# codeslake/RefVSR

Hardware: AMD Instinct MI355X
Metric: 4x SR frames/sec (270p->1080p, RefVSR_small_L1) (higher is better)
Workload: dtype f16; 1 GPU; config_RefVSR_small_L1 4x SR, 270x480 -> 1080x1920, frame_num=5, steady-state sliding window, n=1 (BASELINE configs[1]); synthetic clip seed 0, seeded random weights 1234; frames_per_rank=20, parallelism=frame-shard x1 (reset-aligned, no collective), window_cache=True, frame_ids=True, pipelined_calls=True, frames_per_call=4, headline_mode=frame groups, pipe_layout=pfm, full=False

## Files before the change

### refvsr_amd/csrc/common.h

```cpp
#pragma once
#include <stdlib.h>
#include <hip/hip_runtime.h>
#include <hip/hip_fp16.h>
#include <stdint.h>
#include <stdio.h>
#include <string.h>
#include <type_traits>
#include <utility>

#include "../../include/refvsr_hip.h"

typedef _Float16 f16;
typedef f16 f16x2 __attribute__((ext_vector_type(2)));
typedef f16 f16x4 __attribute__((ext_vector_type(4)));
typedef f16 f16x8 __attribute__((ext_vector_type(8)));
typedef float f32x4 __attribute__((ext_vector_type(4)));
typedef float f32x16 __attribute__((ext_vector_type(16)));

void refvsr_set_error(const char* fmt, ...);

#define RV_CHECK(cond, ...)                        \
    do {                                           \
        if (!(cond)) {                             \
            refvsr_set_error(__VA_ARGS__);         \
            return 1;                              \
        }                                          \
    } while (0)

#define RV_HIP(call)                                                                  \
    do {                                                                              \
        hipError_t e_ = (call);                                                       \
        if (e_ != hipSuccess) {                                                       \
            refvsr_set_error("%s failed: %s (%s:%d)", #call, hipGetErrorString(e_), __FILE__, __LINE__); \
            return 2;                                                                 \
        }                                                                             \
    } while (0)

#define RV_LAUNCH_CHECK() RV_HIP(hipGetLastError())

static inline int rv_cdiv(int a, int b) { return (a + b - 1) / b; }

template <class F, int... I>
__device__ __forceinline__ void rv_static_for(F&& f, std::integer_sequence<int, I...>) { (f(std::integral_constant<int, I>{}), ...); }

#define RV_MAX_DEVICES 16
static inline int rv_device() {
    int d = 0;
    if (hipGetDevice(&d) != hipSuccess || d < 0 || d >= RV_MAX_DEVICES) d = 0;
    return d;
}
static inline int rv_num_cus() {
    static int n_cu[RV_MAX_DEVICES] = {};
    const int d = rv_device();
    if (n_cu[d] == 0) {
        hipDeviceProp_t prop;
        if (hipGetDeviceProperties(&prop, d) == hipSuccess) n_cu[d] = prop.multiProcessorCount;
        if (n_cu[d] <= 0) n_cu[d] = 256;
    }
    return n_cu[d];
}

int rv_stream_cus(hipStream_t st);

struct RvLaunchCap {
    bool attr_done[RV_MAX_DEVICES];
    int occ[RV_MAX_DEVICES];
    size_t occ_lds[RV_MAX_DEVICES];
};
template <typename Kernel>
static int rv_launch_cap(RvLaunchCap& c, Kernel kernel, int block, size_t attr_lds, size_t lds, hipStream_t st, int* cap) {
    const int dev = rv_device();
    if (!c.attr_done[dev]) {
        RV_HIP(hipFuncSetAttribute(reinterpret_cast<const void*>(kernel), hipFuncAttributeMaxDynamicSharedMemorySize, (int)attr_lds));
        c.attr_done[dev] = true;
    }
    if (block == 0) {
        c.occ[dev] = 1;
    } else if (c.occ[dev] == 0 || c.occ_lds[dev] != lds) {
        int occ = 0;
        RV_HIP(hipOccupancyMaxActiveBlocksPerMultiprocessor(&occ, kernel, block, lds));
        c.occ[dev] = occ < 1 ? 1 : occ;
        c.occ_lds[dev] = lds;
    }
    *cap = (rv_stream_cus(st) * c.occ[dev]) & ~7;
    if (*cap < 8) *cap = 8;
    return 0;
}

template <typename Args, typename Launch>
static int rv_resblock_chain(const char* name, int pxb, int min_blob, const void* const* src, int batch, int h, int w, int n,
                             const void* blobs, size_t blob_stride, float act_slope, void* scratch0, void* scratch1, void* const* out,
                             void* stream, Launch launch) {
    RV_CHECK(src && out && blobs && h > 0 && w > 0 && n >= 1 && batch >= 1 && batch <= REFVSR_MAX_MAPS, "%s: bad args", name);
    RV_CHECK(blob_stride >= (size_t)min_blob && blob_stride % 16 == 0 && ((uintptr_t)blobs & 15) == 0,
             "%s: blobs must be 16-byte aligned, stride >= %d", name, min_blob);
    RV_CHECK(act_slope >= 0.f && act_slope <= 1.f, "%s: activation slope must lie in [0, 1]", name);
    RV_CHECK(n == 1 || scratch0, "%s: n >= 2 needs scratch0", name);
    RV_CHECK(n <= 2 || scratch1, "%s: n >= 3 needs scratch1", name);
    const size_t mapb = (size_t)h * w * pxb;
    for (int b = 0; b < batch; ++b) {
        RV_CHECK(src[b] && out[b], "%s: null map pointer (map %d)", name, b);
        for (int c = 0; c < batch; ++c) {
            const unsigned char* s0 = scratch0 ? (const unsigned char*)scratch0 + c * mapb : nullptr;
            const unsigned char* s1 = scratch1 ? (const unsigned char*)scratch1 + c * mapb : nullptr;
            RV_CHECK(src[b] != out[c] && s0 != out[b] && s1 != out[b] && (n < 2 || s0 != src[b]) && (n < 3 || s1 != src[b]) &&
                     (c == b || out[b] != out[c]), "%s: buffers must be distinct", name);
        }
    }
    RV_CHECK(n < 3 || scratch0 != scratch1, "%s: buffers must be distinct", name);
    RV_CHECK((long long)h * w * pxb < (1ll << 31), "%s: map too large for 32-bit offsets", name);
    RV_CHECK(refvsr_init() == 0, "init failed");
    Args a;
    memset(&a, 0, sizeof(a));
    a.h = h; a.w = w; a.act_slope = act_slope; a.batch = batch;
    hipStream_t st = (hipStream_t)stream;
    const unsigned char* cur[REFVSR_MAX_MAPS];
    for (int b = 0; b < batch; ++b) cur[b] = (const unsigned char*)src[b];
    for (int i = 0; i < n; ++i) {
        unsigned char* sc = (unsigned char*)((i & 1) ? scratch1 : scratch0);
        for (int b = 0; b < batch; ++b) {
            a.bsrc[b] = cur[b];
            a.bout[b] = (i == n - 1) ? (unsigned char*)out[b] : sc + b * mapb;
        }
        a.src = a.bsrc[0]; a.out = a.bout[0]; a.blob = (const unsigned char*)blobs + (size_t)i * blob_stride;
        const int rc = launch(a, st);
        if (rc) return rc;
        for (int b = 0; b < batch; ++b) cur[b] = a.bout[b];
    }
    return 0;
}

__device__ __forceinline__ void rv_tile_range(const int n_tiles, const int g, int& t_begin, int& t_end) {
    const int b = (int)blockIdx.x;
    int rank = b;
    if (g >= 8) {
        const int xcd = b & 7;
        rank = b >> 3;
        for (int y = 0; y < xcd; ++y) rank += (g - y + 7) >> 3;
    }
    const unsigned un = (unsigned)n_tiles, ug = (unsigned)g;
    t_begin = (int)(((unsigned)rank * un) / ug);
    t_end = (int)(((unsigned)(rank + 1) * un) / ug);
}

__device__ __forceinline__ int rv_reflect(int i, int n) {
    i = i < 0 ? -i : i;
    return i >= n ? 2 * (n - 1) - i : i;
}

__device__ __forceinline__ float rv_lrelu(float v, float slope) { return v >= 0.f ? v : v * slope; }

__device__ __forceinline__ float rv_linspace_m1p1(int j, int n) {
    const float step = 2.0f / (float)(n - 1);
    return (j < n / 2) ? (-1.0f + step * (float)j) : (1.0f - step * (float)(n - 1 - j));
}

struct WarpCoord { int x0, y0; float w00, w01, w10, w11; bool v00, v01, v10, v11; };

__device__ __forceinline__ WarpCoord warp_coord_uv(const float u, const float v, int hf, int wf, int hin, int win, int y, int x);
__device__ __forceinline__ WarpCoord warp_coord(const float* flow, int hf, int wf, int hin, int win, int y, int x) {
    const size_t fp = (size_t)y * wf + x;
    return warp_coord_uv(flow[fp], flow[(size_t)hf * wf + fp], hf, wf, hin, win, y, x);
}
__device__ __forceinline__ WarpCoord warp_coord_uv(const float u, const float v, int hf, int wf, int hin, int win, int y, int x) {
    const float gx = rv_linspace_m1p1(x, wf) + u / (((float)win - 1.0f) / 2.0f);
    const float gy = rv_linspace_m1p1(y, hf) + v / (((float)hin - 1.0f) / 2.0f);
    const float xs = ((gx + 1.0f) * (float)win - 1.0f) / 2.0f;
    const float ys = ((gy + 1.0f) * (float)hin - 1.0f) / 2.0f;
    const float fx = floorf(xs), fy = floorf(ys);
    const float tx = xs - fx, ty = ys - fy;
    WarpCoord c;
    c.x0 = (int)fminf(fmaxf(fx, -2.0f), (float)win + 1.0f);
    c.y0 = (int)fminf(fmaxf(fy, -2.0f), (float)hin + 1.0f);
    const bool xin0 = c.x0 >= 0 && c.x0 < win, xin1 = c.x0 + 1 >= 0 && c.x0 + 1 < win;
    const bool yin0 = c.y0 >= 0 && c.y0 < hin, yin1 = c.y0 + 1 >= 0 && c.y0 + 1 < hin;
    c.v00 = xin0 && yin0; c.v01 = xin1 && yin0; c.v10 = xin0 && yin1; c.v11 = xin1 && yin1;
    c.w00 = (1.0f - ty) * (1.0f - tx); c.w01 = (1.0f - ty) * tx;
    c.w10 = ty * (1.0f - tx); c.w11 = ty * tx;
    return c;
}

__device__ __forceinline__ uint4 warp_group16(const unsigned char* x, int pixb, int hin, int win, const WarpCoord& c, int goff) {
    float acc[8] = {0, 0, 0, 0, 0, 0, 0, 0};
    auto tap = [&](bool valid, int yy, int xx, float wgt) {
        if (valid) {
            const f16x8 v = *reinterpret_cast<const f16x8*>(x + ((size_t)yy * win + xx) * pixb + goff);
#pragma unroll
            for (int k = 0; k < 8; ++k) acc[k] += wgt * (float)v[k];
        }
    };
    tap(c.v00, c.y0, c.x0, c.w00);
    tap(c.v01, c.y0, c.x0 + 1, c.w01);
    tap(c.v10, c.y0 + 1, c.x0, c.w10);
    tap(c.v11, c.y0 + 1, c.x0 + 1, c.w11);
    union { f16x8 h; uint4 u; } o;
#pragma unroll
    for (int k = 0; k < 8; ++k) o.h[k] = (f16)acc[k];
    return o.u;
}

__device__ __forceinline__ void rv_bilinear_ac_src(int o, int n_in, int n_out, int& i0, int& i1, float& l1) {
#pragma clang fp contract(off)
    const float sc = n_out > 1 ? (float)(n_in - 1) / (float)(n_out - 1) : 0.0f;
    const float x = (float)o * sc;
    i0 = min((int)x, n_in - 1);
    i1 = min(i0 + 1, n_in - 1);
    l1 = x - (float)i0;
}
__device__ __forceinline__ float rv_bilinear_ac2_at(const float* __restrict__ s, int h, int w, int oy, int ox) {
    int y0, y1, x0, x1;
    float ly, lx;
    rv_bilinear_ac_src(oy, h, 2 * h, y0, y1, ly);
    rv_bilinear_ac_src(ox, w, 2 * w, x0, x1, lx);
    const float wy0 = 1.0f - ly, wx0 = 1.0f - lx;
    const float r0 = fmaf(lx, s[(size_t)y0 * w + x1], fmaf(wx0, s[(size_t)y0 * w + x0], 0.0f));
    const float r1 = fmaf(lx, s[(size_t)y1 * w + x1], fmaf(wx0, s[(size_t)y1 * w + x0], 0.0f));
    return fmaf(ly, r1, fmaf(wy0, r0, 0.0f));
}

__device__ __forceinline__ void rv_cubic_taps(float t, float* wgt) {
    const float A = -0.75f;
    float x = t + 1.0f;
    wgt[0] = ((A * x - 5.0f * A) * x + 8.0f * A) * x - 4.0f * A;
    x = t;
    wgt[1] = ((A + 2.0f) * x - (A + 3.0f)) * x * x + 1.0f;
    x = 1.0f - t;
    wgt[2] = ((A + 2.0f) * x - (A + 3.0f)) * x * x + 1.0f;
    x = 2.0f - t;
    wgt[3] = ((A * x - 5.0f * A) * x + 8.0f * A) * x - 4.0f * A;
}
__device__ __forceinline__ void rv_cubic_src(int o, int n_in, float scale, int* idx, float* wgt) {
    const float x = ((float)o + 0.5f) * scale - 0.5f;
    const float fl = floorf(x);
    const int ix = (int)fl;
    rv_cubic_taps(x - fl, wgt);
#pragma unroll
    for (int k = 0; k < 4; ++k) idx[k] = min(max(ix - 1 + k, 0), n_in - 1);
}
__device__ __forceinline__ float rv_bicubic_at(const float* __restrict__ s, int h, int w, int oy, int ox, float sy, float sx) {
    int iy[4], ix[4];
    float wy[4], wx[4];
    rv_cubic_src(oy, h, sy, iy, wy);
    rv_cubic_src(ox, w, sx, ix, wx);
    float acc = 0.0f;
#pragma unroll
    for (int j = 0; j < 4; ++j) {
        float r = 0.0f;
        const float* row = s + (size_t)iy[j] * w;
#pragma unroll
        for (int i = 0; i < 4; ++i) r = fmaf(wx[i], row[ix[i]], r);
        acc = fmaf(wy[j], r, acc);
    }
    return acc;
}

__device__ __forceinline__ void rv_store_result(void* out, const size_t e, const float v, const int fmt) {
    const int f = fmt & REFVSR_RESULT_FMT_MASK;
    if (f == REFVSR_RESULT_F32) reinterpret_cast<float*>(out)[e] = v;
    else if (f == REFVSR_RESULT_F16) reinterpret_cast<f16*>(out)[e] = (f16)v;
    else reinterpret_cast<unsigned char*>(out)[e] = (unsigned char)__float2int_rn(v * 255.0f);
}
__host__ __device__ __forceinline__ size_t rv_result_index(const int fmt, const int c, const int y, const int x, const int h, const int w) {
    return (fmt & REFVSR_RESULT_HWC) ? ((size_t)y * w + x) * 3 + c : ((size_t)c * h + y) * w + x;
}
static inline bool rv_result_fmt_ok(const int fmt) {
    return fmt >= 0 && (fmt & ~(REFVSR_RESULT_FMT_MASK | REFVSR_RESULT_HWC)) == 0 && (fmt & REFVSR_RESULT_FMT_MASK) <= REFVSR_RESULT_U8;
}

__host__ __device__ inline int rv_keven(int ks, int ncg) {
    const int ce = (ncg + 1) >> 1, co = ncg >> 1;
    return ks * (((ks + 1) >> 1) * ce + (ks >> 1) * co);
}
__host__ __device__ inline int rv_ksteps(int ks, int ncg) { return (ks * ks * ncg + (rv_keven(ks, ncg) & 1) + 3) / 4; }
__host__ __device__ inline int rv_kslot(int ty, int tx, int cg, int ks, int ncg) {
    const int ce = (ncg + 1) >> 1, co = ncg >> 1;
    const int p = (tx + cg) & 1;
    const int c0 = p ? co : ce, c1 = p ? ce : co;
    const int row = ((ks + 1) >> 1) * c0 + (ks >> 1) * c1;
    const int rank = ty * row + ((tx + 1) >> 1) * c0 + (tx >> 1) * c1 + (cg >> 1);
    if (!p) return rank;
    const int E = rv_keven(ks, ncg);
    return E + (E & 1) + rank;
}
__host__ __device__ inline int rv_kpad_slot(int j, int ks, int ncg) {
    const int E = rv_keven(ks, ncg);
    return ((E & 1) && j == 0) ? E : ks * ks * ncg + j;
}
__device__ __forceinline__ int rv_pix16(int n) { return (n < 4 || n >= 12) ? ((n & 7) << 1) : (((n - 4) << 1) | 1); }
```

### refvsr_amd/csrc/conv24.hip

```cpp
#include "common.h"
#include "conv24_plan.h"
#include <stdlib.h>

struct C24Args {
    const unsigned char* src0; const unsigned char* src1; unsigned char* out;
    const unsigned char* blob; const unsigned char* mul; const unsigned char* res;
    int h, w, tiles_x, n_tiles, grid;
    float act_slope, post_slope;
    const float* conf_a; const float* conf_b;
    const float* cw0; const float* cb0;
    float* conf_max;
    int ch, cw;
    float slope0;
    const float* base_lr; int bh, bw; float base_step;
    int out_fmt;
    int batch, tpm;
    const unsigned char* bsrc0[REFVSR_MAX_MAPS]; const unsigned char* bsrc1[REFVSR_MAX_MAPS]; unsigned char* bout[REFVSR_MAX_MAPS];
    const unsigned char* bmul[REFVSR_MAX_MAPS]; const unsigned char* bres[REFVSR_MAX_MAPS];
    const float* bconf_a[REFVSR_MAX_MAPS]; const float* bconf_b[REFVSR_MAX_MAPS]; float* bconf_max[REFVSR_MAX_MAPS];
};

constexpr int c24_nf(int cout, int wf) { return wf ? (cout == 24 ? 2 : cout / 16) : cout == 24 ? 3 : cout == 3 ? 1 : cout / 8; }

__device__ __forceinline__ float c24_fold1(const float a) {
    const unsigned u = __float_as_uint(a);
    const auto pr = __builtin_amdgcn_permlane32_swap(u, u, false, false);
    const unsigned x0 = pr[0], x1 = pr[1];
    return __uint_as_float(x0) + __uint_as_float(x1);
}

template <int COUT, int NCG0, int NCG1, int NWV, int TH, int WPS, int SHUF = 0, int CONF = 0, int HALF = 0, int MM = 0, int WF = 0>
__global__ __launch_bounds__(NWV * 64) __attribute__((amdgpu_waves_per_eu(WPS, WPS))) void conv24_kernel(C24Args p) {
    static_assert(WF == 0 || COUT != 3, "output head: one fragment in either format");
    static_assert(HALF == 0 || (COUT == 24 && SHUF == 0 && CONF == 0), "channel-half variant: 24 computed channels per workgroup");
    static_assert(MM == 0 || (HALF == 0 && COUT != 3), "multi-map variant");
    static_assert(SHUF == 0 || (COUT == 48 && (SHUF == 24 || SHUF == 48) && NCG0 * 8 == SHUF && NCG1 == 0), "pixel-shuffle variant");
    static_assert(CONF == 0 || (NCG0 == 2 && NCG1 == 0 && SHUF == 0), "confidence variant: 16-channel single source");
    constexpr int NCG = NCG0 + NCG1, PS = NCG | 1, PXB = PS * 16, ROWB = C24_XW * PXB;
    constexpr int S = c24_steps(NCG), NPAT = c24_npat(NCG);
    constexpr int NF = c24_nf(COUT, WF);
    constexpr int NM = COUT == 24 ? 2 : COUT == 3 ? 1 : COUT / 16;
    constexpr int BIASB = COUT == 48 ? 256 : 128;
    constexpr int WB = S * NF * 1024, BIAS = WB, XT = WB + BIASB;
    constexpr int NT = NWV * 64, T = 2 * TH / NWV;
    constexpr int C24_TH = TH, C24_XH = TH + 2, C24_NPX = C24_XH * C24_XW;
    constexpr int NCH = C24_NPX * NCG, KCH = (NCH + NT - 1) / NT;
    constexpr int PIXB0 = NCG0 * 16, PIXB1 = NCG1 * 16;
    constexpr int OPX = HALF ? 96 : COUT * 2;
    static_assert((COUT == 3 || COUT == 24 || COUT == 32 || COUT == 48) && S > 0 && T >= 1 && T * NWV == 2 * TH, "unsupported shape");
    static_assert(COUT != 3 || (NCG1 == 0 && SHUF == 0 && CONF == 0), "output head: single source");
    extern __shared__ __attribute__((aligned(16))) unsigned char smem[];

    asm volatile("" :: "s"(p.src0), "s"(p.src1), "s"(p.out), "s"(p.blob), "s"(p.mul), "s"(p.res), "s"(p.h), "s"(p.w), "s"(p.tiles_x),
                 "s"(p.n_tiles), "s"(p.grid), "s"(p.act_slope), "s"(p.post_slope));
    const int tid = threadIdx.x;
    const int lane = tid & 63;
    const int wave = __builtin_amdgcn_readfirstlane(tid >> 6);

    {
        constexpr int NPC = WB / 1024;
        const unsigned char* g = p.blob + ((SHUF || HALF) ? (int)blockIdx.y * (WB + BIASB) : 0) + lane * 16;
#pragma unroll
        for (int j = 0; j < (NPC + NWV - 1) / NWV; ++j) {
            const int c = wave + j * NWV;
            if (c < NPC)
                __builtin_amdgcn_global_load_lds((const __attribute__((address_space(1))) void*)(g + c * 1024),
                                                 (__attribute__((address_space(3))) void*)(smem + c * 1024), 16, 0, 0);
        }
        if (wave == NPC % NWV && lane < BIASB / 16)
            __builtin_amdgcn_global_load_lds((const __attribute__((address_space(1))) void*)(g + NPC * 1024),
                                             (__attribute__((address_space(3))) void*)(smem + NPC * 1024), 16, 0, 0);
    }

    if constexpr (HALF != 0) {
        const int zoff = (int)blockIdx.y * 48;
        p.out += zoff;
        if (p.mul) p.mul += zoff;
        if (p.res) p.res += zoff;
    }
    const int rowp = p.w;
    unsigned xg[KCH], xl[KCH];
    unsigned xs1 = 0;
#pragma unroll
    for (int k = 0; k < KCH; ++k) {
        const int i = min(tid + k * NT, NCH - 1);
        const int px = i / NCG, cg = i - px * NCG;
        const int r = px / C24_XW, c = px - r * C24_XW;
        const bool s1 = cg >= NCG0;
        xg[k] = (unsigned)((r * rowp + c) * (s1 ? PIXB1 : PIXB0) + (s1 ? cg - NCG0 : cg) * 16);
        xl[k] = (unsigned)(XT + px * PXB + cg * 16);
        xs1 |= s1 ? (1u << k) : 0u;
    }
    uint4 xv[KCH];
    auto x_fetch = [&](const int tf) {
        int t = tf;
        const unsigned char* s0p = p.src0;
        const unsigned char* s1p = p.src1;
        if constexpr (MM != 0) {
            const int bm = (int)((unsigned)tf / (unsigned)p.tpm);
            t = tf - bm * p.tpm;
            s0p = p.bsrc0[bm];
            if constexpr (NCG1 != 0) s1p = p.bsrc1[bm];
        }
        const int tyi = t / p.tiles_x;
        const int ty0 = tyi * C24_TH, tx0 = (t - tyi * p.tiles_x) * C24_TW;
        const bool interior = ty0 >= 1 && ty0 + C24_TH + 1 <= p.h && tx0 >= 1 && tx0 + C24_TW + 1 <= p.w;
        const long long org = (long long)(ty0 - 1) * p.w + (tx0 - 1);
        const unsigned char* b0 = s0p + org * PIXB0;
        const unsigned char* b1 = NCG1 ? s1p + org * PIXB1 : b0;
        if (interior) {
#pragma unroll
            for (int k = 0; k < KCH; ++k)
                xv[k] = *reinterpret_cast<const uint4*>((NCG1 && ((xs1 >> k) & 1) ? b1 : b0) + xg[k]);
        } else {
            int tide = tid;
            asm volatile("" : "+v"(tide));
#pragma unroll
            for (int k = 0; k < KCH; ++k) {
                const int i = min(tide + k * NT, NCH - 1);
                const int px = i / NCG, cg = i - px * NCG;
                const int r = px / C24_XW, c = px - r * C24_XW;
                const int iy = ty0 - 1 + r, ix = tx0 - 1 + c;
                const bool ok = (unsigned)iy < (unsigned)p.h && (unsigned)ix < (unsigned)p.w;
                const bool s1 = cg >= NCG0;
                const unsigned pix = (unsigned)(min(max(iy, 0), p.h - 1) * p.w + min(max(ix, 0), p.w - 1));
                const unsigned char* g = s1 ? s1p + pix * PIXB1 + (cg - NCG0) * 16 : s0p + pix * PIXB0 + cg * 16;
                uint4 v = *reinterpret_cast<const uint4*>(g);
                const unsigned keep = ok ? 0xffffffffu : 0u;
                v.x &= keep; v.y &= keep; v.z &= keep; v.w &= keep;
                xv[k] = v;
            }
        }
    };
    auto x_park = [&]() {
#pragma unroll
        for (int k = 0; k < KCH; ++k)
            if (k * NT + NT <= NCH || tid + k * NT < NCH) *reinterpret_cast<uint4*>(smem + xl[k]) = xv[k];
    };
    constexpr int PTH = TH + 4, PTW = C24_XW + 2;
    constexpr int PT = XT + C24_NPX * PXB, CW0 = PT + 2 * PTH * PTW * 4, CB0 = CW0 + 18 * 16 * 4;
    if constexpr (CONF != 0) {
        float* wl0 = reinterpret_cast<float*>(smem + CW0);
        for (int i = tid; i < 18 * 16; i += NT) {
            const int co = i & 15, tap = i >> 4;
            wl0[i] = p.cw0[(co * 2 + tap / 9) * 9 + tap % 9];
        }
        if (tid < 16) reinterpret_cast<float*>(smem + CB0)[tid] = p.cb0[tid];
    }
    auto conf_stage = [&](const int tf) {
        int t = tf;
        const float* cap = p.conf_a;
        const float* cbp = p.conf_b;
        float* cmp_ = p.conf_max;
        if constexpr (MM != 0) {
            const int bm = (int)((unsigned)tf / (unsigned)p.tpm);
            t = tf - bm * p.tpm;
            cap = p.bconf_a[bm]; cbp = p.bconf_b[bm];
            if (p.conf_max) cmp_ = p.bconf_max[bm];
        }
        const int tyi = t / p.tiles_x;
        const int ty0 = tyi * C24_TH, tx0 = (t - tyi * p.tiles_x) * C24_TW;
        float* pt = reinterpret_cast<float*>(smem + PT);
        for (int i = tid; i < 2 * PTH * PTW; i += NT) {
            const int c = i / (PTH * PTW), rem = i - c * (PTH * PTW);
            const int r = rem / PTW, cc = rem - r * PTW;
            const int y = ty0 - 2 + r, x = tx0 - 2 + cc;
            float v = 0.0f;
            if ((unsigned)y < (unsigned)p.h && (unsigned)x < (unsigned)p.w) {
                const float* src = c ? cbp : cap;
                if constexpr (CONF == 1) v = src[(size_t)y * p.cw + x];
                else v = fminf(fmaxf(rv_bicubic_at(src, p.ch, p.cw, y, x, 0.5f, 0.5f), 0.0f), 1.0f);
            }
            pt[i] = v;
        }
        __syncthreads();
        const float* wl0 = reinterpret_cast<const float*>(smem + CW0);
        const float* bl0 = reinterpret_cast<const float*>(smem + CB0);
#pragma unroll
        for (int k = 0; k < KCH; ++k) {
            const int i = tid + k * NT;
            if (i < NCH) {
                const int px = i >> 1, cg = i & 1;
                const int r = px / C24_XW, c = px - r * C24_XW;
                const int iy = ty0 - 1 + r, ix = tx0 - 1 + c;
                uint4 v = make_uint4(0u, 0u, 0u, 0u);
                if ((unsigned)iy < (unsigned)p.h && (unsigned)ix < (unsigned)p.w) {
                    float acc[8] = {0.f, 0.f, 0.f, 0.f, 0.f, 0.f, 0.f, 0.f};
#pragma unroll
                    for (int ci = 0; ci < 2; ++ci)
#pragma unroll
                        for (int ky = 0; ky < 3; ++ky)
#pragma unroll
                            for (int kx = 0; kx < 3; ++kx) {
                                const float xv = pt[ci * (PTH * PTW) + (r + ky) * PTW + (c + kx)];
                                const f32x4 w0 = *reinterpret_cast<const f32x4*>(wl0 + (ci * 9 + ky * 3 + kx) * 16 + cg * 8);
                                const f32x4 w1 = *reinterpret_cast<const f32x4*>(wl0 + (ci * 9 + ky * 3 + kx) * 16 + cg * 8 + 4);
                                acc[0] = fmaf(xv, w0[0], acc[0]); acc[1] = fmaf(xv, w0[1], acc[1]);
                                acc[2] = fmaf(xv, w0[2], acc[2]); acc[3] = fmaf(xv, w0[3], acc[3]);
                                acc[4] = fmaf(xv, w1[0], acc[4]); acc[5] = fmaf(xv, w1[1], acc[5]);
                                acc[6] = fmaf(xv, w1[2], acc[6]); acc[7] = fmaf(xv, w1[3], acc[7]);
                            }
                    union { f16x8 h; uint4 u; } o;
#pragma unroll
                    for (int j = 0; j < 8; ++j) o.h[j] = (f16)rv_lrelu(acc[j] + bl0[cg * 8 + j], p.slope0);
                    v = o.u;
                }
                *reinterpret_cast<uint4*>(smem + XT + px * PXB + cg * 16) = v;
            }
        }
        if constexpr (CONF == 1) {
            if (p.conf_max) {
                for (int i = tid; i < C24_TH * C24_TW; i += NT) {
                    const int r = i / C24_TW, c = i - r * C24_TW;
                    const int y = ty0 + r, x = tx0 + c;
                    if (y < p.h && x < p.w)
                        cmp_[(size_t)y * p.w + x] = fmaxf(pt[(r + 2) * PTW + c + 2], pt[PTH * PTW + (r + 2) * PTW + c + 2]);
                }
            }
        }
    };
    int tl, k_hi;
    rv_tile_range(p.n_tiles, p.grid, tl, k_hi);
    if constexpr (CONF == 0) { if (tl < k_hi) x_fetch(tl); }
    __builtin_amdgcn_sched_barrier(0);

    const int q = lane >> 4;
    const int lp = rv_pix16(lane & 15);
    const int la = lane * 16;
    const int g0w = wave * T;
#define RW(t) ((g0w + (t)) >> 1)
#define CG(t) ((g0w + (t)) & 1)
    auto sel4 = [&](const int v0, const int v1, const int v2, const int v3) { return q == 0 ? v0 : q == 1 ? v1 : q == 2 ? v2 : v3; };
    int pb[T];
#pragma unroll
    for (int t = 0; t < T; ++t)
        pb[t] = XT + RW(t) * ROWB + (CG(t) * 16 + lp) * PXB +
                sel4(c24_off(NCG, 0, 0), c24_off(NCG, 0, 1), c24_off(NCG, 0, 2), c24_off(NCG, 0, 3)) - c24_off(NCG, 0, 0);
    int pd[NPAT];
#pragma unroll
    for (int pp = 0; pp < NPAT; ++pp) {
        const int s = c24_pat_step(NCG, pp);
        pd[pp] = (sel4(c24_off(NCG, s, 0), c24_off(NCG, s, 1), c24_off(NCG, s, 2), c24_off(NCG, s, 3)) - c24_off(NCG, s, 0)) -
                 (sel4(c24_off(NCG, 0, 0), c24_off(NCG, 0, 1), c24_off(NCG, 0, 2), c24_off(NCG, 0, 3)) - c24_off(NCG, 0, 0));
    }
    const int rowb_o = p.w * OPX;
    const unsigned oo = (unsigned)(lp * OPX + q * 8);

    if constexpr (CONF == 0) { if (tl < k_hi) x_park(); }
    __syncthreads();

    for (; tl < k_hi; ++tl) {
        const bool has_next = tl + 1 < k_hi;
        if constexpr (CONF != 0) {
            conf_stage(tl);
            __syncthreads();
        }
        int tm = tl;
        unsigned char* outp = p.out;
        const unsigned char* mulp = p.mul;
        const unsigned char* resp = p.res;
        if constexpr (MM != 0) {
            const int bm = (int)((unsigned)tl / (unsigned)p.tpm);
            tm = tl - bm * p.tpm;
            outp = p.bout[bm];
            if (p.mul) mulp = p.bmul[bm];
            if (p.res) resp = p.bres[bm];
        }
        const int tyi = tm / p.tiles_x;
        const int ty0 = tyi * C24_TH, tx0 = (tm - tyi * p.tiles_x) * C24_TW;
        const bool interior = ty0 >= 1 && ty0 + C24_TH + 1 <= p.h && tx0 >= 1 && tx0 + C24_TW + 1 <= p.w;
        const long long oorg = ((long long)ty0 * p.w + tx0) * OPX;
        f16x4 mv[NM][T], rv[NM][T];
        bool okt[T];
#pragma unroll
        for (int t = 0; t < T; ++t) {
            okt[t] = true;
            if (!interior) {
                int lpe = lp;
                asm volatile("" : "+v"(lpe));
                okt[t] = ty0 + RW(t) < p.h && tx0 + CG(t) * 16 + lpe < p.w;
            }
            const unsigned eo = (unsigned)(RW(t) * rowb_o) + oo + CG(t) * 16 * OPX;
#pragma unroll
            for (int m = 0; m < NM; ++m) {
                mv[m][t] = rv[m][t] = (f16x4){(f16)0.f, (f16)0.f, (f16)0.f, (f16)0.f};
                const bool lane_ok = okt[t] && (COUT != 24 || m == 0 || q < 2);
                if constexpr (COUT == 24) {
                    if (p.mul && lane_ok) mv[m][t] = *reinterpret_cast<const f16x4*>(mulp + oorg + eo + 32 * m);
                    if (p.res && lane_ok) rv[m][t] = *reinterpret_cast<const f16x4*>(resp + oorg + eo + 32 * m);
                }
                (void)lane_ok;
            }
        }
        if constexpr (CONF == 0) { if (has_next) x_fetch(tl + 1); }

        f32x4 acc[NM][T];
#pragma unroll
        for (int m = 0; m < NM; ++m) {
            const f32x4 bv = *reinterpret_cast<const f32x4*>(smem + BIAS + m * 64 + q * 16);
#pragma unroll
            for (int t = 0; t < T; ++t) acc[m][t] = bv;
        }
        {
            uint4 fa[2][NF], fb[2][T];
            auto load = [&](auto sc, uint4 (&af)[NF], uint4 (&bf)[T]) {
                constexpr int s = decltype(sc)::value;
                constexpr int pp = c24_pat(NCG, s);
                constexpr int imm = c24_off(NCG, s, 0);
#pragma unroll
                for (int f = 0; f < NF; ++f) af[f] = *reinterpret_cast<const uint4*>(smem + (s * NF + f) * 1024 + la);
#pragma unroll
                for (int t = 0; t < T; ++t) {
                    if constexpr (pp == 0) bf[t] = *reinterpret_cast<const uint4*>(smem + pb[t] + imm);
                    else bf[t] = *reinterpret_cast<const uint4*>(smem + pb[t] + pd[pp] + imm);
                }
            };
            auto mfma = [&](const uint4 (&af)[NF], const uint4 (&bf)[T]) {
                if constexpr (WF == 1) {
#pragma unroll
                    for (int m = 0; m < NM; ++m) {
                        const f16x8 av = *reinterpret_cast<const f16x8*>(&af[m]);
#pragma unroll
                        for (int t = 0; t < T; ++t)
                            acc[m][t] = __builtin_amdgcn_mfma_f32_16x16x32_f16(av, *reinterpret_cast<const f16x8*>(&bf[t]), acc[m][t], 0, 0, 0);
                    }
                } else if constexpr (COUT == 24) {
                    const f16x8 a_hi = *reinterpret_cast<const f16x8*>(&af[0]);
                    const f16x8 a_lo = *reinterpret_cast<const f16x8*>(&af[1]);
                    const f16x8 a_mx = *reinterpret_cast<const f16x8*>(&af[2]);
#pragma unroll
                    for (int t = 0; t < T; ++t) acc[0][t] = __builtin_amdgcn_mfma_f32_16x16x32_f16(a_hi, *reinterpret_cast<const f16x8*>(&bf[t]), acc[0][t], 0, 0, 0);
#pragma unroll
                    for (int t = 0; t < T; ++t) acc[1][t] = __builtin_amdgcn_mfma_f32_16x16x32_f16(a_mx, *reinterpret_cast<const f16x8*>(&bf[t]), acc[1][t], 0, 0, 0);
#pragma unroll
                    for (int t = 0; t < T; ++t) acc[0][t] = __builtin_amdgcn_mfma_f32_16x16x32_f16(a_lo, *reinterpret_cast<const f16x8*>(&bf[t]), acc[0][t], 0, 0, 0);
                } else if constexpr (COUT == 3) {
                    const f16x8 a_w = *reinterpret_cast<const f16x8*>(&af[0]);
#pragma unroll
                    for (int t = 0; t < T; ++t) acc[0][t] = __builtin_amdgcn_mfma_f32_16x16x32_f16(a_w, *reinterpret_cast<const f16x8*>(&bf[t]), acc[0][t], 0, 0, 0);
                } else {
#pragma unroll
                    for (int h = 0; h < 2; ++h)
#pragma unroll
                        for (int m = 0; m < NM; ++m) {
                            const f16x8 av = *reinterpret_cast<const f16x8*>(&af[2 * m + h]);
#pragma unroll
                            for (int t = 0; t < T; ++t)
                                acc[m][t] = __builtin_amdgcn_mfma_f32_16x16x32_f16(av, *reinterpret_cast<const f16x8*>(&bf[t]), acc[m][t], 0, 0, 0);
                        }
                }
            };
            if constexpr (NF <= 4) {
                load(std::integral_constant<int, 0>{}, fa[0], fb[0]);
                rv_static_for([&](auto sc) {
                    constexpr int s = decltype(sc)::value;
                    if constexpr (s + 1 < S) load(std::integral_constant<int, s + 1>{}, fa[(s + 1) & 1], fb[(s + 1) & 1]);
                    __builtin_amdgcn_sched_barrier(0);
                    mfma(fa[s & 1], fb[s & 1]);
                }, std::make_integer_sequence<int, S>{});
            } else {
                load(std::integral_constant<int, 0>{}, fa[0], fb[0]);
                rv_static_for([&](auto sc) {
                    constexpr int s = decltype(sc)::value;
                    __builtin_amdgcn_sched_barrier(0);
                    mfma(fa[0], fb[0]);
                    __builtin_amdgcn_sched_barrier(0);
                    if constexpr (s + 1 < S) load(std::integral_constant<int, s + 1>{}, fa[0], fb[0]);
                }, std::make_integer_sequence<int, S>{});
            }
        }
        if (has_next) {
            __syncthreads();
            if constexpr (CONF == 0) x_park();
        }
        if constexpr (COUT == 3) {
            const size_t plane_b = (size_t)p.bh * p.bw;
#pragma unroll
            for (int t = 0; t < T; ++t) {
                const f32x4 y = acc[0][t];
                const float s0 = c24_fold1(y[0]), s1 = c24_fold1(y[1]), s2 = c24_fold1(y[2]);
                const int srcl = lane & 15;
                const float v0 = __shfl(s0, srcl), v1 = __shfl(s1, srcl), v2 = __shfl(s2, srcl);
                const float v = q == 0 ? v0 : q == 1 ? v1 : v2;
                int lpe = lp;
                if (!interior) asm volatile("" : "+v"(lpe));
                const int oy = ty0 + RW(t), ox = tx0 + CG(t) * 16 + lpe;
                if (q < 3 && oy < p.h && ox < p.w) {
                    const float b = fminf(fmaxf(rv_bicubic_at(p.base_lr + q * plane_b, p.bh, p.bw, oy, ox, p.base_step, p.base_step), 0.0f), 1.0f);
                    rv_store_result(outp, rv_result_index(p.out_fmt, q, oy, ox, p.h, p.w), fminf(fmaxf(v + b, 0.0f), 1.0f), p.out_fmt);
                }
            }
        } else if constexpr (SHUF != 0) {
            const int z = (int)blockIdx.y;
            const unsigned w2 = 2u * (unsigned)p.w;
#pragma unroll
            for (int t = 0; t < T; ++t) {
                int lpe = lp;
                if (!interior) asm volatile("" : "+v"(lpe));
                const unsigned oy = (unsigned)(ty0 + RW(t)), ox = (unsigned)(tx0 + CG(t) * 16 + lpe);
#pragma unroll
                for (int m = 0; m < NM; ++m) {
                    const int r0 = 16 * m + 4 * q;
                    const int dx = SHUF == 24 ? (r0 >= 24 ? 1 : 0) : (z & 1);
                    const int dy = SHUF == 24 ? z : (z >> 1);
                    const int ch0 = SHUF == 24 ? r0 - 24 * dx : r0;
                    f32x4 y = acc[m][t];
                    if (p.act_slope != 1.0f) {
#pragma unroll
                        for (int i = 0; i < 4; ++i) y[i] = fmaxf(y[i], y[i] * p.act_slope);
                    }
                    const f16x4 o = {(f16)y[0], (f16)y[1], (f16)y[2], (f16)y[3]};
                    if (okt[t])
                        *reinterpret_cast<f16x4*>(outp + ((2u * oy + dy) * w2 + 2u * ox + dx) * (unsigned)(SHUF * 2) + ch0 * 2) = o;
                }
            }
        } else
        {
            unsigned char* ob = outp + oorg;
#pragma unroll
            for (int t = 0; t < T; ++t) {
                unsigned char* d = ob + (unsigned)(RW(t) * rowb_o) + oo + CG(t) * 16 * OPX;
#pragma unroll
                for (int m = 0; m < NM; ++m) {
                    f32x4 y = acc[m][t];
                    if constexpr (COUT == 24) {
                        if (WF == 0 && m == 1) y = (f32x4){c24_fold1(y[0]), c24_fold1(y[1]), c24_fold1(y[2]), c24_fold1(y[3])};
                    } else {
                        const unsigned eo = (unsigned)(RW(t) * rowb_o) + oo + CG(t) * 16 * OPX;
                        if (p.mul && okt[t]) mv[m][t] = *reinterpret_cast<const f16x4*>(mulp + oorg + eo + 32 * m);
                        if (p.res && okt[t]) rv[m][t] = *reinterpret_cast<const f16x4*>(resp + oorg + eo + 32 * m);
                    }
                    if (p.act_slope != 1.0f) {
#pragma unroll
                        for (int i = 0; i < 4; ++i) y[i] = fmaxf(y[i], y[i] * p.act_slope);
                    }
                    if (p.mul) {
#pragma unroll
                        for (int i = 0; i < 4; ++i) y[i] *= (float)mv[m][t][i];
                    }
                    if (p.res) {
#pragma unroll
                        for (int i = 0; i < 4; ++i) y[i] += (float)rv[m][t][i];
                    }
                    if (p.post_slope != 1.0f) {
#pragma unroll
                        for (int i = 0; i < 4; ++i) y[i] = fmaxf(y[i], y[i] * p.post_slope);
                    }
                    const f16x4 o = {(f16)y[0], (f16)y[1], (f16)y[2], (f16)y[3]};
                    if (okt[t] && (COUT != 24 || m == 0 || q < 2)) *reinterpret_cast<f16x4*>(d + 32 * m) = o;
                }
            }
        }
        if constexpr (CONF == 0) { if (has_next) __syncthreads(); }
    }
#undef RW
#undef CG
}

template <int COUT, int NCG0, int NCG1, int NWV, int TH, int WPS, int SHUF = 0, int CONF = 0, int HALF = 0, int MM = 0, int WF = 0>
static int launch_c24(C24Args& a, hipStream_t st) {
    constexpr int NZ = HALF ? 2 : SHUF == 0 ? 1 : SHUF == 24 ? 2 : 4;
    constexpr int NCG = NCG0 + NCG1, PS = NCG | 1;
    constexpr int LDS = c24_steps(NCG) * c24_nf(COUT, WF) * 1024 + (COUT == 48 ? 256 : 128) + (TH + 2) * C24_XW * PS * 16 +
                        (CONF ? 2 * (TH + 4) * (C24_XW + 2) * 4 + 18 * 16 * 4 + 64 : 0);
    static_assert(LDS <= 160 * 1024, "LDS budget");
    static bool attr_done[RV_MAX_DEVICES] = {};
    static int occ_dev[RV_MAX_DEVICES] = {};
    const int dev = rv_device();
    if (!attr_done[dev]) {
        RV_HIP(hipFuncSetAttribute(reinterpret_cast<const void*>(&conv24_kernel<COUT, NCG0, NCG1, NWV, TH, WPS, SHUF, CONF, HALF, MM, WF>),
                                   hipFuncAttributeMaxDynamicSharedMemorySize, LDS));
        int occ = 0;
        RV_HIP(hipOccupancyMaxActiveBlocksPerMultiprocessor(&occ, conv24_kernel<COUT, NCG0, NCG1, NWV, TH, WPS, SHUF, CONF, HALF, MM, WF>, NWV * 64, LDS));
        occ_dev[dev] = occ < 1 ? 1 : occ;
        attr_done[dev] = true;
    }
    a.tiles_x = rv_cdiv(a.w, C24_TW);
    a.tpm = a.tiles_x * rv_cdiv(a.h, TH);
    a.n_tiles = a.tpm * (MM ? a.batch : 1);
    int cap = (rv_stream_cus(st) * occ_dev[dev] / NZ) & ~7;
    if (cap < 8) cap = 8;
    a.grid = a.n_tiles < cap ? a.n_tiles : cap;
    hipLaunchKernelGGL((conv24_kernel<COUT, NCG0, NCG1, NWV, TH, WPS, SHUF, CONF, HALF, MM, WF>), dim3(a.grid, NZ), dim3(NWV * 64), LDS, st, a);
    RV_LAUNCH_CHECK();
    return 0;
}

extern "C" int refvsr_conv24_supported(int c0, int c1) {
    return (c0 == 24 && c1 == 0) || (c0 == 16 && c1 == 0) || (c0 == 8 && c1 == 24) || (c0 == 24 && c1 == 24);
}
extern "C" int refvsr_conv48_supported(int c0, int c1) {
    return (c0 == 48 && c1 == 0) || (c0 == 16 && c1 == 0) || (c0 == 48 && c1 == 48) || (c0 == 8 && c1 == 48);
}
extern "C" int refvsr_conv32_supported(int c0, int c1) { return (c0 == 32 && c1 == 0) || (c0 == 8 && c1 == 0); }

extern "C" int refvsr_conv24_blob_bytes(int c0, int c1) {
    if (!refvsr_conv24_supported(c0, c1)) return -1;
    return c24_steps((c0 + c1) / 8) * 3 * 1024 + 128;
}
extern "C" int refvsr_conv32_blob_bytes(int c0, int c1) {
    if (!refvsr_conv32_supported(c0, c1)) return -1;
    return c24_steps((c0 + c1) / 8) * 4 * 1024 + 128;
}
extern "C" int refvsr_conv48_blob_bytes(int c0, int c1) {
    if (!refvsr_conv48_supported(c0, c1)) return -1;
    if (c0 == 48 && c1 == 48) return 2 * (c24_steps(12) * 3 * 1024 + 128);
    return c24_steps((c0 + c1) / 8) * 6 * 1024 + 256;
}

extern "C" int refvsr_conv_shuffle2_supported(int c) { return c == 24 || c == 48; }
extern "C" int refvsr_conv_shuffle2_blob_bytes(int c) {
    if (!refvsr_conv_shuffle2_supported(c)) return -1;
    return (c == 24 ? 2 : 4) * (c24_steps(c / 8) * 6 * 1024 + 256);
}

extern "C" int refvsr_conv24_f16w_blob_bytes(int c0, int c1) {
    if (!refvsr_conv24_supported(c0, c1)) return -1;
    return c24_steps((c0 + c1) / 8) * c24_nf(24, 1) * 1024 + 128;
}
extern "C" int refvsr_conv32_f16w_blob_bytes(int c0, int c1) {
    if (!refvsr_conv32_supported(c0, c1)) return -1;
    return c24_steps((c0 + c1) / 8) * c24_nf(32, 1) * 1024 + 128;
}
extern "C" int refvsr_conv_shuffle2_f16w_blob_bytes(int c) {
    if (c != 24) return -1;
    return 2 * (c24_steps(c / 8) * c24_nf(48, 1) * 1024 + 256);
}

extern "C" int refvsr_conv24_kblock(int ncg, int s, int q) {
    if (c24_steps(ncg) == 0 || s < 0 || s >= c24_steps(ncg) || q < 0 || q > 3) return -2;
    return c24_kblock(ncg, s, q);
}

static int c24_fill(C24Args& a, const char* who, int cout, const void* src0, const void* src1, int c1, int h, int w, const void* blob,
                    float act_slope, const void* mul, const void* res, float post_slope, void* out) {
    RV_CHECK(src0 && out && blob && h > 0 && w > 0, "%s: bad args", who);
    RV_CHECK((c1 == 0) == (src1 == nullptr), "%s: src1 / c1 mismatch", who);
    RV_CHECK(((uintptr_t)blob & 15) == 0, "%s: blob must be 16-byte aligned", who);
    RV_CHECK(act_slope >= 0.f && act_slope <= 1.f && post_slope >= 0.f && post_slope <= 1.f, "%s: activation slopes must lie in [0, 1]", who);
    RV_CHECK(src0 != out && src1 != out, "%s: in-place operation is not supported", who);
    RV_CHECK((long long)h * w * cout * 2 < (1ll << 31), "%s: map too large for 32-bit offsets", who);
    RV_CHECK(refvsr_init() == 0, "init failed");
    memset(&a, 0, sizeof(a));
    a.src0 = (const unsigned char*)src0; a.src1 = (const unsigned char*)src1; a.out = (unsigned char*)out;
    a.blob = (const unsigned char*)blob; a.mul = (const unsigned char*)mul; a.res = (const unsigned char*)res;
    a.h = h; a.w = w; a.act_slope = act_slope; a.post_slope = post_slope;
    return 0;
}

static int c24_fill_maps(C24Args& a, const char* who, int cout, const void* const* src0, const void* const* src1, int c1, int batch,
                         int h, int w, const void* blob, float act_slope, const void* const* mul, const void* const* res,
                         float post_slope, void* const* out) {
    if (c24_fill(a, who, cout, src0[0], src1 ? src1[0] : nullptr, c1, h, w, blob, act_slope, mul ? mul[0] : nullptr,
                 res ? res[0] : nullptr, post_slope, out[0])) return 1;
    a.batch = batch;
    for (int b = 0; b < batch; ++b) {
        RV_CHECK(src0[b] && out[b] && (!src1 || src1[b]) && (!mul || mul[b]) && (!res || res[b]), "%s: null map pointer (map %d)", who, b);
        for (int c = 0; c < batch; ++c)
            RV_CHECK(src0[c] != out[b] && (!src1 || src1[c] != out[b]) && (c == b || out[c] != out[b]), "%s: in-place operation is not supported", who);
        a.bsrc0[b] = (const unsigned char*)src0[b]; a.bsrc1[b] = src1 ? (const unsigned char*)src1[b] : nullptr;
        a.bout[b] = (unsigned char*)out[b];
        a.bmul[b] = mul ? (const unsigned char*)mul[b] : nullptr; a.bres[b] = res ? (const unsigned char*)res[b] : nullptr;
    }
    return 0;
}
#define C24_OPT(p) ((p) ? &(p) : nullptr)

template <int WF, int MM>
static int c24_conv24(const void* const* src0, int c0, const void* const* src1, int c1, int batch, int h, int w, const void* blob,
                      float act_slope, const void* const* mul, const void* const* res, float post_slope, void* const* out, void* stream) {
    const char* who = MM ? "conv24_batch" : "conv24";
    RV_CHECK(refvsr_conv24_supported(c0, c1), "%s: %d + %d input channels not supported", who, c0, c1);
    RV_CHECK(src0 && out && batch >= 1 && batch <= REFVSR_MAX_MAPS, "%s: 1..%d maps per launch", who, REFVSR_MAX_MAPS);
    RV_CHECK(!MM || (c1 == 0) == (src1 == nullptr), "%s: src1 / c1 mismatch", who);
    C24Args a;
    if (c24_fill_maps(a, who, 24, src0, src1, c1, batch, h, w, blob, act_slope, mul, res, post_slope, out)) return 1;
    hipStream_t st = (hipStream_t)stream;
    if (c0 == 24 && c1 == 0) return launch_c24<24, 3, 0, 8, 8, 4, 0, 0, 0, MM, WF>(a, st);
    if (c0 == 16 && c1 == 0) return launch_c24<24, 2, 0, 8, 8, 4, 0, 0, 0, MM, WF>(a, st);
    if (c0 == 8 && c1 == 24) return launch_c24<24, 1, 3, 8, 8, 4, 0, 0, 0, MM, WF>(a, st);
    return launch_c24<24, 3, 3, 8, 8, 4, 0, 0, 0, MM, WF>(a, st);
}
#define C24_CONV_ARGS const void* src0, int c0, const void* src1, int c1, int h, int w, const void* blob, float act_slope, \
                      const void* mul, const void* res, float post_slope, void* out, void* stream
#define C24_CONV_BATCH_ARGS const void* const* src0, int c0, const void* const* src1, int c1, int batch, int h, int w, const void* blob, \
                            float act_slope, const void* const* mul, const void* const* res, float post_slope, void* const* out, void* stream
#define C24_CONV_PASS(MM, WF) c24_conv24<WF, MM>(&src0, c0, C24_OPT(src1), c1, 1, h, w, blob, act_slope, C24_OPT(mul), C24_OPT(res), post_slope, &out, stream)
#define C24_CONV_BATCH_PASS(WF) c24_conv24<WF, 1>(src0, c0, src1, c1, batch, h, w, blob, act_slope, mul, res, post_slope, out, stream)
extern "C" int refvsr_conv24(C24_CONV_ARGS) { return C24_CONV_PASS(0, 0); }
extern "C" int refvsr_conv24_f16w(C24_CONV_ARGS) { return C24_CONV_PASS(0, 1); }
extern "C" int refvsr_conv24_batch(C24_CONV_BATCH_ARGS) { return C24_CONV_BATCH_PASS(0); }
extern "C" int refvsr_conv24_batch_f16w(C24_CONV_BATCH_ARGS) { return C24_CONV_BATCH_PASS(1); }

template <int WF>
static int c24i_conv32(C24_CONV_ARGS) {
    RV_CHECK(refvsr_conv32_supported(c0, c1), "conv32: %d + %d input channels not supported", c0, c1);
    C24Args a;
    if (c24_fill(a, "conv32", 32, src0, src1, c1, h, w, blob, act_slope, mul, res, post_slope, out)) return 1;
    hipStream_t st = (hipStream_t)stream;
    if (c0 == 32) return launch_c24<32, 4, 0, 8, 8, 4, 0, 0, 0, 0, WF>(a, st);
    return launch_c24<32, 1, 0, 8, 8, 4, 0, 0, 0, 0, WF>(a, st);
}
extern "C" int refvsr_conv32(C24_CONV_ARGS) { return c24i_conv32<0>(src0, c0, src1, c1, h, w, blob, act_slope, mul, res, post_slope, out, stream); }
extern "C" int refvsr_conv32_f16w(C24_CONV_ARGS) { return c24i_conv32<1>(src0, c0, src1, c1, h, w, blob, act_slope, mul, res, post_slope, out, stream); }

extern "C" int refvsr_conv48(C24_CONV_ARGS) {
    RV_CHECK(refvsr_conv48_supported(c0, c1), "conv48: %d + %d input channels not supported", c0, c1);
    C24Args a;
    if (c24_fill(a, "conv48", 48, src0, src1, c1, h, w, blob, act_slope, mul, res, post_slope, out)) return 1;
    hipStream_t st = (hipStream_t)stream;
    static const bool w8 = getenv("REFVSR_CONV48_WAVES") && atoi(getenv("REFVSR_CONV48_WAVES")) == 8;
    if (c0 == 48 && c1 == 48) return launch_c24<24, 6, 6, 16, 8, 4, 0, 0, 1>(a, st);
    if (c0 == 8 && c1 == 48) return launch_c24<48, 1, 6, 16, 8, 4>(a, st);
    if (c0 == 48) return w8 ? launch_c24<48, 6, 0, 8, 16, 2>(a, st) : launch_c24<48, 6, 0, 16, 16, 4>(a, st);
    return launch_c24<48, 2, 0, 8, 8, 4>(a, st);
}

// ... 82 lines not shown
```

Baseline: 237.1 frames/s.

## Prefetch confidence inputs across tiles and restructure fused first-conv stage

The confidence variant of the conv24 kernel now prefetches its confidence-map inputs for the next tile into registers during the current tile's MMA work (c_fetch/c_park), like the existing x_fetch pipeline. The 2x bicubic upsample is rewritten to work on a staged low-res window in LDS using separable polyphase taps, instead of a full 16-tap gather per output pixel. The first 2->16 conv is reassigned so each wave computes one output-channel pair over 6-pixel strips with weights held in registers, using inline-asm FMAs. The cost is more LDS, more registers and a hard requirement of 8 waves with TH=8.

```diff
diff --git a/refvsr_amd/csrc/common.h b/refvsr_amd/csrc/common.h
--- a/refvsr_amd/csrc/common.h
+++ b/refvsr_amd/csrc/common.h
@@ -148,6 +148,11 @@
     return i >= n ? 2 * (n - 1) - i : i;
 }
 
+__device__ __forceinline__ float rv_fma1(const float a, const float b, float c) {
+    asm("v_fmac_f32_e32 %0, %1, %2" : "+v"(c) : "v"(a), "v"(b));
+    return c;
+}
+
 __device__ __forceinline__ float rv_lrelu(float v, float slope) { return v >= 0.f ? v : v * slope; }
 
 __device__ __forceinline__ float rv_linspace_m1p1(int j, int n) {
@@ -237,6 +242,10 @@
 #pragma unroll
     for (int k = 0; k < 4; ++k) idx[k] = min(max(ix - 1 + k, 0), n_in - 1);
 }
+__device__ __forceinline__ void rv_cubic_phase_taps(int o, float scale, float* wgt) {
+    const float x = ((float)o + 0.5f) * scale - 0.5f;
+    rv_cubic_taps(x - floorf(x), wgt);
+}
 __device__ __forceinline__ float rv_bicubic_at(const float* __restrict__ s, int h, int w, int oy, int ox, float sy, float sx) {
     int iy[4], ix[4];
     float wy[4], wx[4];
diff --git a/refvsr_amd/csrc/conv24.hip b/refvsr_amd/csrc/conv24.hip
--- a/refvsr_amd/csrc/conv24.hip
+++ b/refvsr_amd/csrc/conv24.hip
@@ -138,74 +138,152 @@
             if (k * NT + NT <= NCH || tid + k * NT < NCH) *reinterpret_cast<uint4*>(smem + xl[k]) = xv[k];
     };
     constexpr int PTH = TH + 4, PTW = C24_XW + 2;
-    constexpr int PT = XT + C24_NPX * PXB, CW0 = PT + 2 * PTH * PTW * 4, CB0 = CW0 + 18 * 16 * 4;
+    constexpr int SWH = TH / 2 + 6, SWW = C24_TW / 2 + 6;
+    constexpr int PT = XT + C24_NPX * PXB, CW0 = PT + 2 * PTH * PTW * 4, CB0 = CW0 + 18 * 16 * 4, SW = CB0 + 64;
+    static_assert(CONF == 0 || (NWV == 8 && TH == 8), "confidence variant: eight waves, one channel pair of the first conv each");
     if constexpr (CONF != 0) {
         float* wl0 = reinterpret_cast<float*>(smem + CW0);
         for (int i = tid; i < 18 * 16; i += NT) {
-            const int co = i & 15, tap = i >> 4;
-            wl0[i] = p.cw0[(co * 2 + tap / 9) * 9 + tap % 9];
+            const int cp = i / 36, rem = i - cp * 36;
+            wl0[i] = p.cw0[(2 * cp + (rem & 1)) * 18 + (rem >> 1)];
         }
         if (tid < 16) reinterpret_cast<float*>(smem + CB0)[tid] = p.cb0[tid];
     }
-    auto conf_stage = [&](const int tf) {
+    constexpr int NCV = CONF == 1 ? (2 * PTH * PTW + NT - 1) / NT : 1;
+    constexpr int NCI = CONF == 1 ? 2 * PTH * PTW : 2 * SWH * SWW;
+    float cv[NCV];
+    auto c_fetch = [&](const int tf) {
         int t = tf;
         const float* cap = p.conf_a;
         const float* cbp = p.conf_b;
+        if constexpr (MM != 0) {
+            const int bm = (int)((unsigned)tf / (unsigned)p.tpm);
+            t = tf - bm * p.tpm;
+            cap = p.bconf_a[bm]; cbp = p.bconf_b[bm];
+        }
+        const int tyi = t / p.tiles_x;
+        const int ty0 = tyi * C24_TH, tx0 = (t - tyi * p.tiles_x) * C24_TW;
+        constexpr int WH = CONF == 1 ? PTH : SWH, WW = CONF == 1 ? PTW : SWW;
+        int tide = tid;
+        asm volatile("" : "+v"(tide));
+#pragma unroll
+        for (int k = 0; k < NCV; ++k) {
+            const int i = min(tide + k * NT, NCI - 1);
+            const int cf_m = i / (WH * WW), rem = i - cf_m * (WH * WW);
+            const int cf_r = rem / WW, cf_c = rem - cf_r * WW;
+            const float* src = cf_m ? cbp : cap;
+            if constexpr (CONF == 1) {
+                const int y = ty0 - 2 + cf_r, x = tx0 - 2 + cf_c;
+                const bool ok = (unsigned)y < (unsigned)p.h && (unsigned)x < (unsigned)p.w;
+                const float v = src[(size_t)min(max(y, 0), p.h - 1) * p.cw + min(max(x, 0), p.w - 1)];
+                cv[k] = ok ? v : 0.0f;
+            } else {
+                const int y = min(max((ty0 >> 1) - 3 + cf_r, 0), p.ch - 1), x = min(max((tx0 >> 1) - 3 + cf_c, 0), p.cw - 1);
+                cv[k] = src[(size_t)y * p.cw + x];
+            }
+        }
+    };
+    auto c_park = [&]() {
+        float* dst = reinterpret_cast<float*>(smem + (CONF == 1 ? PT : SW));
+#pragma unroll
+        for (int k = 0; k < NCV; ++k)
+            if (tid + k * NT < NCI) dst[tid + k * NT] = cv[k];
+    };
+    auto conf_stage = [&](const int tf) {
+        int t = tf;
         float* cmp_ = p.conf_max;
         if constexpr (MM != 0) {
             const int bm = (int)((unsigned)tf / (unsigned)p.tpm);
             t = tf - bm * p.tpm;
-            cap = p.bconf_a[bm]; cbp = p.bconf_b[bm];
             if (p.conf_max) cmp_ = p.bconf_max[bm];
         }
         const int tyi = t / p.tiles_x;
         const int ty0 = tyi * C24_TH, tx0 = (t - tyi * p.tiles_x) * C24_TW;
         float* pt = reinterpret_cast<float*>(smem + PT);
-        for (int i = tid; i < 2 * PTH * PTW; i += NT) {
-            const int c = i / (PTH * PTW), rem = i - c * (PTH * PTW);
-            const int r = rem / PTW, cc = rem - r * PTW;
-            const int y = ty0 - 2 + r, x = tx0 - 2 + cc;
-            float v = 0.0f;
-            if ((unsigned)y < (unsigned)p.h && (unsigned)x < (unsigned)p.w) {
-                const float* src = c ? cbp : cap;
-                if constexpr (CONF == 1) v = src[(size_t)y * p.cw + x];
-                else v = fminf(fmaxf(rv_bicubic_at(src, p.ch, p.cw, y, x, 0.5f, 0.5f), 0.0f), 1.0f);
-            }
-            pt[i] = v;
-        }
-        __syncthreads();
-        const float* wl0 = reinterpret_cast<const float*>(smem + CW0);
-        const float* bl0 = reinterpret_cast<const float*>(smem + CB0);
-#pragma unroll
-        for (int k = 0; k < KCH; ++k) {
-            const int i = tid + k * NT;
-            if (i < NCH) {
-                const int px = i >> 1, cg = i & 1;
-                const int r = px / C24_XW, c = px - r * C24_XW;
-                const int iy = ty0 - 1 + r, ix = tx0 - 1 + c;
-                uint4 v = make_uint4(0u, 0u, 0u, 0u);
-                if ((unsigned)iy < (unsigned)p.h && (unsigned)ix < (unsigned)p.w) {
-                    float acc[8] = {0.f, 0.f, 0.f, 0.f, 0.f, 0.f, 0.f, 0.f};
-#pragma unroll
-                    for (int ci = 0; ci < 2; ++ci)
-#pragma unroll
-                        for (int ky = 0; ky < 3; ++ky)
-#pragma unroll
-                            for (int kx = 0; kx < 3; ++kx) {
-                                const float xv = pt[ci * (PTH * PTW) + (r + ky) * PTW + (c + kx)];
-                                const f32x4 w0 = *reinterpret_cast<const f32x4*>(wl0 + (ci * 9 + ky * 3 + kx) * 16 + cg * 8);
-                                const f32x4 w1 = *reinterpret_cast<const f32x4*>(wl0 + (ci * 9 + ky * 3 + kx) * 16 + cg * 8 + 4);
-                                acc[0] = fmaf(xv, w0[0], acc[0]); acc[1] = fmaf(xv, w0[1], acc[1]);
-                                acc[2] = fmaf(xv, w0[2], acc[2]); acc[3] = fmaf(xv, w0[3], acc[3]);
-                                acc[4] = fmaf(xv, w1[0], acc[4]); acc[5] = fmaf(xv, w1[1], acc[5]);
-                                acc[6] = fmaf(xv, w1[2], acc[6]); acc[7] = fmaf(xv, w1[3], acc[7]);
-                            }
-                    union { f16x8 h; uint4 u; } o;
-#pragma unroll
-                    for (int j = 0; j < 8; ++j) o.h[j] = (f16)rv_lrelu(acc[j] + bl0[cg * 8 + j], p.slope0);
-                    v = o.u;
-                }
-                *reinterpret_cast<uint4*>(smem + XT + px * PXB + cg * 16) = v;
+        int tide = tid;
+        asm volatile("" : "+v"(tide));
+        if constexpr (CONF == 2) {
+            if (tide < 2 * (PTH / 2) * (PTW / 2)) {
+                float cwe[4], cwo[4];
+                int o = 0;
+                asm volatile("" : "+v"(o));
+                rv_cubic_phase_taps(o, 0.5f, cwe);
+                rv_cubic_phase_taps(o + 1, 0.5f, cwo);
+                const int m = tide / ((PTH / 2) * (PTW / 2)), rem = tide - m * ((PTH / 2) * (PTW / 2));
+                const int f = rem / (PTW / 2), e = rem - f * (PTW / 2);
+                const int s1_src = m * (SWH * SWW) + f * SWW + e, s1_dst = m * (PTH * PTW) + 2 * f * PTW + 2 * e;
+                const int s1_y = 2 * f - 2, s1_x = 2 * e - 2;
+                const float* s = reinterpret_cast<const float*>(smem + SW) + s1_src;
+                float hs[5][2];
+#pragma unroll
+                for (int a = 0; a < 5; ++a) {
+                    float v[5];
+#pragma unroll
+                    for (int i = 0; i < 5; ++i) v[i] = s[a * SWW + i];
+                    float r = 0.0f;
+#pragma unroll
+                    for (int i = 0; i < 4; ++i) r = fmaf(cwe[i], v[i], r);
+                    hs[a][0] = r;
+                    r = 0.0f;
+#pragma unroll
+                    for (int i = 0; i < 4; ++i) r = fmaf(cwo[i], v[i + 1], r);
+                    hs[a][1] = r;
+                }
+#pragma unroll
+                for (int py = 0; py < 2; ++py) {
+                    float o2[2];
+#pragma unroll
+                    for (int px = 0; px < 2; ++px) {
+                        float acc = 0.0f;
+#pragma unroll
+                        for (int j = 0; j < 4; ++j) acc = fmaf(py ? cwo[j] : cwe[j], hs[py + j][px], acc);
+                        const int y = ty0 + s1_y + py, x = tx0 + s1_x + px;
+                        const bool ok = (unsigned)y < (unsigned)p.h && (unsigned)x < (unsigned)p.w;
+                        o2[px] = ok ? fminf(fmaxf(acc, 0.0f), 1.0f) : 0.0f;
+                    }
+                    *reinterpret_cast<float2*>(pt + s1_dst + py * PTW) = make_float2(o2[0], o2[1]);
+                }
+            }
+            __syncthreads();
+        }
+        const int lane_ = tide & 63;
+        if (lane_ < 60) {
+            const int s2_r = lane_ / 6, s2_c = (lane_ - s2_r * 6) * 6;
+            float wr[36];
+#pragma unroll
+            for (int i = 0; i < 9; ++i) {
+                const f32x4 w4 = *reinterpret_cast<const f32x4*>(smem + CW0 + wave * 144 + i * 16);
+                wr[4 * i] = w4[0]; wr[4 * i + 1] = w4[1]; wr[4 * i + 2] = w4[2]; wr[4 * i + 3] = w4[3];
+            }
+            float acc[6][2];
+#pragma unroll
+            for (int j = 0; j < 6; ++j) acc[j][0] = acc[j][1] = 0.0f;
+#pragma unroll
+            for (int ci = 0; ci < 2; ++ci)
+#pragma unroll
+                for (int ky = 0; ky < 3; ++ky) {
+                    const float2* rowp = reinterpret_cast<const float2*>(pt + ci * (PTH * PTW) + (s2_r + ky) * PTW + s2_c);
+                    float xw[8];
+#pragma unroll
+                    for (int i = 0; i < 4; ++i) { const float2 v2 = rowp[i]; xw[2 * i] = v2.x; xw[2 * i + 1] = v2.y; }
+#pragma unroll
+                    for (int kx = 0; kx < 3; ++kx)
+#pragma unroll
+                        for (int j = 0; j < 6; ++j) {
+                            acc[j][0] = rv_fma1(xw[j + kx], wr[(ci * 9 + ky * 3 + kx) * 2], acc[j][0]);
+                            acc[j][1] = rv_fma1(xw[j + kx], wr[(ci * 9 + ky * 3 + kx) * 2 + 1], acc[j][1]);
+                        }
+                }
+            const float bs0 = reinterpret_cast<const float*>(smem + CB0)[2 * wave], bs1 = reinterpret_cast<const float*>(smem + CB0)[2 * wave + 1];
+            const int iy = ty0 - 1 + s2_r;
+#pragma unroll
+            for (int j = 0; j < 6; ++j) {
+                const int c = s2_c + j, ix = tx0 - 1 + c;
+                union { f16x2 h; unsigned u; } o;
+                o.h[0] = (f16)rv_lrelu(acc[j][0] + bs0, p.slope0);
+                o.h[1] = (f16)rv_lrelu(acc[j][1] + bs1, p.slope0);
+                const bool ok = (unsigned)iy < (unsigned)p.h && (unsigned)ix < (unsigned)p.w;
+                if (j < 4 || c < C24_XW) *reinterpret_cast<unsigned*>(smem + XT + (s2_r * C24_XW + c) * PXB + wave * 4) = ok ? o.u : 0u;
             }
         }
         if constexpr (CONF == 1) {
@@ -222,6 +300,7 @@
     int tl, k_hi;
     rv_tile_range(p.n_tiles, p.grid, tl, k_hi);
     if constexpr (CONF == 0) { if (tl < k_hi) x_fetch(tl); }
+    else { if (tl < k_hi) c_fetch(tl); }
     __builtin_amdgcn_sched_barrier(0);
 
     const int q = lane >> 4;
@@ -247,6 +326,7 @@
     const unsigned oo = (unsigned)(lp * OPX + q * 8);
 
     if constexpr (CONF == 0) { if (tl < k_hi) x_park(); }
+    else { if (tl < k_hi) c_park(); }
     __syncthreads();
 
     for (; tl < k_hi; ++tl) {
@@ -293,6 +373,7 @@
             }
         }
         if constexpr (CONF == 0) { if (has_next) x_fetch(tl + 1); }
+        else { if (has_next) c_fetch(tl + 1); }
 
         f32x4 acc[NM][T];
 #pragma unroll
@@ -369,9 +450,13 @@
                 }, std::make_integer_sequence<int, S>{});
             }
         }
-        if (has_next) {
-            __syncthreads();
-            if constexpr (CONF == 0) x_park();
+        if constexpr (CONF == 0) {
+            if (has_next) {
+                __syncthreads();
+                x_park();
+            }
+        } else {
+            if (has_next) c_park();
         }
         if constexpr (COUT == 3) {
             const size_t plane_b = (size_t)p.bh * p.bw;
@@ -451,7 +536,7 @@
                 }
             }
         }
-        if constexpr (CONF == 0) { if (has_next) __syncthreads(); }
+        if (has_next) __syncthreads();
     }
 #undef RW
 #undef CG
@@ -462,7 +547,7 @@
     constexpr int NZ = HALF ? 2 : SHUF == 0 ? 1 : SHUF == 24 ? 2 : 4;
     constexpr int NCG = NCG0 + NCG1, PS = NCG | 1;
     constexpr int LDS = c24_steps(NCG) * c24_nf(COUT, WF) * 1024 + (COUT == 48 ? 256 : 128) + (TH + 2) * C24_XW * PS * 16 +
-                        (CONF ? 2 * (TH + 4) * (C24_XW + 2) * 4 + 18 * 16 * 4 + 64 : 0);
+                        (CONF ? 2 * (TH + 4) * (C24_XW + 2) * 4 + 18 * 16 * 4 + 64 : 0) + (CONF == 2 ? 2 * (TH / 2 + 6) * (C24_TW / 2 + 6) * 4 : 0);
     static_assert(LDS <= 160 * 1024, "LDS budget");
     static bool attr_done[RV_MAX_DEVICES] = {};
     static int occ_dev[RV_MAX_DEVICES] = {};
```

Result: no change. 236.7 frames/s, median of 2 (-0.1%).
